# Nightmare-n/GD-MAE

Hardware: AMD Instinct MI355X
Metric: MAE pre-train frames/sec (Waymo-shape, 180k pts, 75% mask) (higher is better)
Workload: dtype bf16

## Files before the change

gd-mae_amd/csrc/decoder_blocks.hip:

```cpp
#include "../../include/gdmae_hip.h"
#include "common.h"
#include "dw_grouped.h"
#include <stdlib.h>

typedef float f32x16 __attribute__((ext_vector_type(16)));
typedef __bf16 bf16x8 __attribute__((ext_vector_type(8)));
typedef short s16x4 __attribute__((ext_vector_type(4)));

namespace {

constexpr int kC = 128;
constexpr int kChunk = 64;
constexpr int kXBytes = kChunk * kC * 2;
constexpr int kMaxTok = 2048;
constexpr int kHP = 6;
constexpr int kQ = 32;

template <int U>
struct Geo {
  static constexpr int TPC = kChunk / (U * U);
  static constexpr int HW = U + 2;
  static constexpr int HS = HW * HW;
  static constexpr int LT = U == 4 ? 36 : 24;
  static constexpr int NP = 2;
// ... 291 lines not shown
  GD_REQUIRE(n < (1ll << 31) && H > 0 && W > 0 && H % u == 0 && W % u == 0, "decoder_block_dw: map size");
  hipStream_t st = (hipStream_t)stream;
  BlockDwArgs A{(const unsigned short*)P, a, b, (const unsigned short*)bg, site, (const unsigned short*)dYc, tile_slot, (float*)workspace,
                n, (int)(n / (u * u)), H, W, (H + 7) / 8, (W + 7) / 8, 0, 0};
  block_dw_pick(n, &A.S, &A.cps);
  GD_REQUIRE(A.S % 8 == 0 && block_dw_fits(u, A.cps), "decoder_block_dw: too many tokens per slice (gdmae_decoder_block_dw_workspace_bytes returns 0)");
  {
    GdTimed timed(GD_T_DEC_CONV_BWD, st, (double)n * (2.0 * kC + 2.0 * kC + 4.0) + 36.0 * A.S * kC * kC, 2.0 * n * 9.0 * kC * kC);
    const int rc = u == 4 ? block_dw_launch<4>(A, st) : block_dw_launch<2>(A, st);
    if (rc) return rc;
  }
  hipLaunchKernelGGL(k_block_dw_reduce, dim3(gd_div_up(9ll * kC * kC, 256)), dim3(256), 0, st, (const float*)workspace, A.S, out, ld_out, m_off);
  GD_LAUNCH_CHECK();
  return 0;
}
```

gd-mae_amd/csrc/plan.hip:

```cpp
#include "../../include/gdmae_hip.h"
#include "common.h"
#include <string.h>

int gd_voxelize_impl(const float* points, long long n_points, int n_cols, const float* lo, const float* vs, const int* grid_xyz,
                     int batch_size, float* points_out, long long* point_coords, long long* inverse, int* inverse32,
                     long long* voxel_coords, int* pillar_cell, int* pillar_pt_off, int* pillar_pts, int* point_rank,
                     int* sample_pillar_off, float* pillar_mean, int* cell2pillar_out, int* counts, void* workspace, size_t workspace_bytes,
                     void* lb_state, float* points_pm, int* row_pillar, hipStream_t st);
size_t gd_voxelize_lb_state_bytes(long long n_points, long long cells);
size_t gd_plan_scan_state_bytes(long long n);
size_t gd_plan_win_state_bytes(long long n);
int gd_plan_visible_tokens(const float* mask, const int* cell2pillar, long long n_cells, int* tok_pillar, int* tok_cell, int* map,
                           int* n_tok, void* lb_state, hipStream_t st);
int gd_plan_downsample(const int* map_in, int B, int Yi, int Xi, int* tok_cell_out, int* map_out, int* n_out, void* lb_state,
                       hipStream_t st);
struct Dims {
  int B, Y, X;
};
struct PlanJob {
  const int* n_tok;
  const int* tok_cell;
  Dims dt, dm;
  const int* map;
  int mode, s;
// ... 74 lines not shown
};

int check(const gdmae_plan_params* p) {
  GD_REQUIRE(p != nullptr, "geometry plan: null parameters");
  GD_REQUIRE(p->n_points >= 0 && p->n_points < (1ll << 31) && p->n_cols >= 4 && p->n_cols <= 65 && p->batch_size >= 1,
             "geometry plan: bad point buffer");
  GD_REQUIRE(p->grid[0] >= 1 && p->grid[1] >= 1 && p->grid[2] == 1, "geometry plan: single-layer pillar grids (spt_backbone_mae.py:94)");
  GD_REQUIRE(p->n_stages >= 1 && p->n_stages <= GDMAE_PLAN_MAX_STAGES, "geometry plan: 1..4 stages");
  for (int i = 0; i < p->n_stages; ++i) {
    GD_REQUIRE(p->stride[i] == 1 || p->stride[i] == 2, "geometry plan: conv_down stride 1 or 2 (k3 s2 p1)");
    GD_REQUIRE(i == 0 || p->stride[i] == 2, "geometry plan: only the first stage may keep the resolution");
    GD_REQUIRE(p->win_x[i] >= 1 && p->win_y[i] >= 1 && p->win_x[i] * p->win_y[i] <= 64, "geometry plan: window must fit one wavefront");
    GD_REQUIRE(p->n_levels[i] >= 1 && p->n_levels[i] <= 3, "geometry plan: 1..3 drop levels");
  }
  GD_REQUIRE(p->n_dec >= 0 && p->n_dec <= 3, "geometry plan: at most 3 decoder source stages");
  for (int g = 0; g < p->n_dec; ++g) GD_REQUIRE(p->dec_sources[g] >= 0 && p->dec_sources[g] < p->n_stages, "geometry plan: decoder source");
  return 0;
}

int layout(const gdmae_plan_params* p, gdmae_plan_buffer* table, int max_entries, Offsets& O, size_t* total, int* n_entries) {
  if (int rc = check(p)) return rc;
  Layout L{table, max_entries, 0, 0, true};
  const int B = p->batch_size, gx = p->grid[0], gy = p->grid[1], F = p->n_cols - 1;
  const long long n0 = p->cap_points > p->n_points ? p->cap_points : p->n_points;
  O.cells = (long long)B * gx * gy;
  GD_REQUIRE(O.cells < (1ll << 31), "geometry plan: B*Y*X must fit int32");
  O.cap_pts = n0 > 0 ? n0 : 1;
  O.m_cap = n0 < O.cells ? n0 : O.cells;
  if (O.m_cap < 1) O.m_cap = 1;
  const long long cap = O.cap_pts;
// ... 71 lines not shown
    if (g.up_s > 1) O.s[i].up_sites = L.add(name("up_sites"), sizeof(int) * g.cap * g.up_s * g.up_s);
    O.s[i].win_ws = L.add(name("win_ws"), gd_plan_windows_ws_bytes(B, g.Y, g.X, p->win_x[i], p->win_y[i]));
    const long long wcap = g.n_win < g.cap ? g.n_win : g.cap;
    for (int sh = 0; sh < 2; ++sh)
      for (int k = 0; k < 7; ++k) {
        snprintf(nm, sizeof(nm), "s%d.w%d.%s", i, sh, kWin[k]);
        O.s[i].w[sh][k] = L.add(nm, sizeof(int) * (k < 5 ? g.cap : wcap));
      }
  }
  O.dec_slot = O.dec_list = O.dec_flag = -1;
  if (O.dec) {
    O.dec_slot = L.add("dec.tile_slot", sizeof(int) * nt);
    O.dec_list = L.add("dec.tile_list", sizeof(int) * nt);
    O.dec_flag = L.add("dec.flag", sizeof(int) * nt);
    for (int g = 0; g < p->n_dec; ++g) {
      const StageGeo& sg = O.geo[p->dec_sources[g]];
      snprintf(nm, sizeof(nm), "dec.nbr%d", g);
      O.dec_nbr[g] = L.add(nm, sizeof(int) * sg.cap * sg.up_s * sg.up_s * 9);
    }
  }
  GD_REQUIRE(L.ok, "geometry plan: buffer table too small");
  if (total) *total = L.off;
  if (n_entries) *n_entries = L.n;
  return 0;
}

}

extern "C" int gdmae_geometry_plan_layout(const gdmae_plan_params* p, gdmae_plan_buffer* table, int max_entries, int* n_entries,
                                          size_t* total_bytes) {
// ... 88 lines not shown
    int rc = gd_plan_jobs(J, cap_max, st);
    if (rc) return rc;
    rc = gd_plan_windows_all(W, ns, st);
    if (rc) return rc;
  }
  if (O.dec) {
    const int* maps[3];
    int ups[3];
    for (int g = 0; g < p->n_dec; ++g) {
      maps[g] = I(O.s[p->dec_sources[g]].map);
      ups[g] = O.geo[p->dec_sources[g]].up_s;
    }
    int rc = gd_decoder_tiles_lb(maps, ups, p->n_dec, B, gy, gx, I(O.dec_slot), I(O.dec_list), n_act, I(O.dec_flag), lb, st);
    if (rc) return rc;
    for (int g = 0; g < p->n_dec; ++g) {
      const int si = p->dec_sources[g];
      const StageGeo& sg = O.geo[si];
      const int* sites = sg.up_s > 1 ? I(O.s[si].up_sites) : I(O.s[si].tok_cell);
      rc = gd_decoder_site_rulebook(sites, n_tok + si, sg.up_s * sg.up_s, sg.cap * sg.up_s * sg.up_s, I(O.dec_slot), gy, gx, I(O.dec_nbr[g]), st);
      if (rc) return rc;
    }
  }
  return 0;
}
```

gd-mae_amd/gdmae_hip/decoder.py:

```python
from __future__ import annotations

import torch
import torch.nn.functional as F

import os

from . import bn as gbn
from . import lib as L
from . import ops, packing
from . import plan as gplan
from . import timing

CONV_BWD = os.environ.get("GDMAE_DEC_BWD", "implicit")
BLOCK_BWD = os.environ.get("GDMAE_DEC_BLOCK", "1")

BN_EPS, BN_MOM = 1e-3, 0.01



def colstats(x2d: torch.Tensor):
    R, C = x2d.shape
    assert x2d.is_contiguous() and x2d.dtype in (torch.float32, torch.bfloat16)
    out = torch.empty(2 * C, dtype=torch.float64, device=x2d.device)
    ws = torch.empty(L.load().gdmae_colstats_workspace_bytes(C), dtype=torch.uint8, device=x2d.device)
    L.call("gdmae_colstats", L.ptr(x2d), R, C, int(x2d.dtype == torch.bfloat16), L.ptr(out), L.ptr(ws), L.stream())
    return out[:C], out[C:]


def _gather_slice(table2d, idx, col0, ncol):
# ... 186 lines not shown
            S = tap_region @ regD
            Wk = conv_w.permute(2, 3, 0, 1).reshape(9, C2, Cin)
            tot = torch.einsum('ko,koi->i', S, Wk.double()).contiguous()
            dWk = (S[:, :, None] * bgz.double()[None, None, :]).float()
            Wd = Wk.to(cdt)
        grads = [None] * 7
        dW_rows = []
        col = 0
        implicit = None
        if (CONV_BWD == "implicit" and tile_slot is not None and y2.dtype == torch.bfloat16 and use_native and C2 == 128
                and all(w == 128 for w in ctx.widths) and len(ctx.geom) > 6 and ctx.geom[6] is not None):
            dt = ctx.geom[6][0]
            packed = packing.decoder_conv_packed(ctx.conv_param, ctx.widths, ctx.direct_w is not None)
            if packed is not None:
                if dt.nbr is None:
                    dt.nbr = gplan.decoder_site_rulebooks(dt, sites, ctx.geom[6][2])
                dYc = torch.empty_like(y2)
                L.call("gdmae_decoder_dy", L.ptr(y2), L.ptr(dt.tile_list), dt.n_act, L.ptr(k01), L.ptr(k01[C2:]), L.ptr(rows),
                       L.ptr(cell2pillar), H, W, C2, L.ptr(dYc), L.stream())
                implicit = (dt, packed, dYc)
        for i, w in enumerate(ctx.widths):
            P = Ps[i]
            n = P.shape[0]
            ab = ab_l[i]
            if implicit is not None:
                dt, packed, dYc = implicit
                nbr = dt.nbr[i]
                assert nbr.shape[0] == n, (nbr.shape, n)
                dX = torch.empty(n, w, dtype=cdt, device=dev)
                L.call("gdmae_spconv", L.ptr(dYc), 0, L.ptr(nbr), packed.data_ptr() + i * 9 * w * C2 * 2, n, C2, w, L.ptr(dX), 8, L.stream())
                bg = bgz[col:col + w]
                u = int(ctx.geom[6][2][i])
                ws_block = 0
                if BLOCK_BWD != "0" and u in (2, 4) and P.dtype == torch.bfloat16 and P.is_contiguous() and sites[i].numel() >= n:
                    ws_block = int(L.load().gdmae_decoder_block_dw_workspace_bytes(n, u))
                if ws_block > 0:
                    ws = torch.empty(ws_block, dtype=torch.uint8, device=dev)
                    L.call("gdmae_decoder_block_dw", L.ptr(P), L.ptr(ab), L.ptr(ab[w:]), L.ptr(bg), L.ptr(sites[i]), n, u, L.ptr(dYc),
                           L.ptr(tile_slot), H, W, L.ptr(dWk), Cin, col, L.ptr(ws), L.stream())
                else:
                    n_pad = int(L.load().gdmae_tap_dw_rows(n, w, C2))
                    Zd = torch.empty(n_pad, w, dtype=cdt, device=dev)
                    L.call("gdmae_rows_affine_relu_sub", L.ptr(P), _bf(P), None, n, w, L.ptr(ab), L.ptr(ab[w:]), L.ptr(bg), L.ptr(Zd),
                           _bf(Zd), w, 0, L.stream())
                    ws = torch.empty(L.load().gdmae_tap_dw_workspace_bytes(n, w, C2), dtype=torch.uint8, device=dev)
                    L.call("gdmae_tap_dw", L.ptr(Zd), n, n_pad, w, L.ptr(dYc), L.ptr(nbr), C2, L.ptr(dWk), Cin, col, L.ptr(ws), L.stream())
            else:
                G = torch.empty(n, 9 * C2, dtype=cdt, device=dev)
                with timing.kernel("k_conv_grad_taps", 2.0 * n * 9 * C2 * G.element_size()):
                    L.call("gdmae_conv3x3_grad_taps", L.ptr(y2), _bf(y2), L.ptr(tile_slot), L.ptr(ybg), L.ptr(k01), L.ptr(k01[C2:]),
# ... 145 lines not shown
        return stage_plan.tok_cell
    pre = getattr(stage_plan, "_up_sites", None)
    if pre is not None and pre[0] == s and stage_plan.Y * s == Y and stage_plan.X * s == X:
        return pre[1]
    return gplan.upsample_cells(stage_plan.tok_cell, stage_plan.Y, stage_plan.X, s).reshape(-1).contiguous()


def sparse_decoder(model_cfg, deblocks, conv_out, hidden, pillar_cell, cell2pillar, B, Y, X, want_dense=False, conv_impl='tiles', pre_conv_hook=None):
    R = B * Y * X
    args, bns = [], []
    cdt = torch.bfloat16 if torch.is_autocast_enabled() else torch.float32
    src_idx = [int(src[-1]) - 1 for src in model_cfg.FEATURES_SOURCE]
    tiles = None
    if cdt == torch.bfloat16 and conv_impl == 'tiles':
        ep = hidden[0]._plan
        dt = gplan.decoder_tiles(ep, src_idx, Y, X)
        tiles = (dt, [hidden[i].stage_plan.map for i in src_idx], [Y // hidden[i].stage_plan.Y for i in src_idx])
    for i, src in enumerate(model_cfg.FEATURES_SOURCE):
        h = hidden[int(src[-1]) - 1]
        sp = h.stage_plan
        deconv, bn = deblocks[i][0], deblocks[i][1]
        s = int(deconv.stride[0])
        assert deconv.kernel_size == (s, s) and sp.Y * s == Y and sp.X * s == X and deconv.bias is None
        P = deconv_rows(h.features, deconv)
        args += [upsampled_sites(sp, s, Y, X), P, bn.weight, bn.bias]
        bns.append(bn)
    conv, bn2 = conv_out[0], conv_out[1]
    outs = DecoderHead.apply((B, Y, X, bns[0].eps, bn2.eps, cdt, tiles, pre_conv_hook), conv.weight, bn2.weight, bn2.bias, pillar_cell,
                             cell2pillar, tuple(bns) + (bn2,), *args)
    out, y2, mean2, var2 = outs[:4]
    dense = None
# ... 22 lines not shown
```

gd-mae_amd/gdmae_hip/lib.py:

```python
from __future__ import annotations

import ctypes as C
import os

import torch

_HERE = os.path.dirname(os.path.abspath(__file__))
LIB_PATH = os.path.abspath(os.path.join(_HERE, "..", "csrc", "libgdmae_hip.so"))
if os.environ.get("GDMAE_LIB"):
    LIB_PATH = os.path.abspath(os.environ["GDMAE_LIB"])


class GdmaeHipError(RuntimeError):
    pass


_P, _I, _L, _F, _D, _Z = C.c_void_p, C.c_int, C.c_longlong, C.c_float, C.c_double, C.c_size_t

SIGNATURES = {
    "gdmae_abi_version": (_I, []),
    "gdmae_target_arch": (C.c_char_p, []),
    "gdmae_last_error": (C.c_char_p, []),
    "gdmae_voxelize_workspace_bytes": (_Z, [_L, _I, _I, _I, _I]),
    "gdmae_voxelize": (_I, [_P, _L, _I, _P, _P, _P, _I, _P, _P, _P, _P, _P, _P, _P, _P, _P, _P, _P, _P, _P, _P, _Z, _P]),
# ... 94 lines not shown
    "gdmae_gemm_tn_splitk": (_I, [_P, _P, _P, _L, _I, _I, _I, _I, _P, _P]),
    "gdmae_conv_block_scratch_bytes": (_Z, [_L, _L, _I, _I, _I]),
    "gdmae_spconv_packed_bytes": (_Z, [_I, _I]),
    "gdmae_spconv_pack_jobs": (_I, [_P, _I, _I, _I, _P, _P]),
    "gdmae_spconv": (_I, [_P, _I, _P, _P, _L, _I, _I, _P, _I, _P]),
    "gdmae_spconv_bias_relu": (_I, [_P, _I, _P, _P, _P, _L, _I, _I, _P, _P]),
    "gdmae_spconv_stat_rows": (_I, [_I, _I, _I]),
    "gdmae_spconv_stats": (_I, [_P, _I, _P, _P, _L, _I, _I, _P, _P, _P]),
    "gdmae_decoder_dy": (_I, [_P, _P, _I, _P, _P, _P, _P, _I, _I, _I, _P, _P]),
    "gdmae_decoder_site_rulebook": (_I, [_P, _P, _I, _L, _P, _I, _I, _P, _P]),
    "gdmae_tap_dw_rows": (_L, [_L, _I, _I]),
    "gdmae_tap_dw_workspace_bytes": (_Z, [_L, _I, _I]),
    "gdmae_tap_dw": (_I, [_P, _L, _L, _I, _P, _P, _I, _P, _I, _I, _P, _P]),
    "gdmae_decoder_block_dw_workspace_bytes": (_Z, [_L, _I]),
    "gdmae_decoder_block_dw": (_I, [_P, _P, _P, _P, _P, _L, _I, _P, _P, _I, _I, _P, _I, _I, _P, _P]),
    "gdmae_conv_block_fwd": (_I, [_P, _P]),
    "gdmae_conv_block_bwd": (_I, [_P, _P]),
    "gdmae_encoder_layer_bytes": (_I, [_L, _I, _I, _I, _I, _P, _P, _P]),
    "gdmae_dw_gemm_workspace_bytes": (_Z, [_L, _I, _I]),
    "gdmae_dw_gemm": (_I, [_P, _P, _L, _I, _I, _P, _P, _P, _P]),
    "gdmae_layer_packed_bytes": (_Z, [_I, _I]),
    "gdmae_layer_pack_jobs": (_I, [_P, _P, _P, _P, _I, _I, _P, _P]),
    "gdmae_layer_pack_job_count": (_I, [_I, _I]),
    "gdmae_tok_gemm_pack": (_I, [_P, _I, _P]),
    "gdmae_tok_gemm": (_I, [_P, _P, _P, _L, _L, _I, _I, _I, _P, _P, _P, _P, _P, _P, _F, _P, _P, _P, _P, _P, _P, _P]),
    "gdmae_tok_gemm_qkv": (_I, [_P, _P, _P, _P, _P, _L, _I, _P, _P, _P]),
    "gdmae_tok_gemm_ffn": (_I, [_P, _P, _P, _P, _P, _L, _L, _I, _P, _P, _P, _P, _F, _P, _P, _P, _P, _P, _P, _P, _P]),
    "gdmae_tok_gemm_ln_bwd_rows": (_I, [_I]),
    "gdmae_tok_gemm_ln_bwd": (_I, [_P, _P, _L, _L, _I, _I, _P, _P, _P, _P, _P, _P, _P, _P, _P, _P]),
    "gdmae_encoder_layer_fwd": (_I, [_P, _P]),
# ... 61 lines not shown
}

class LayerArgs(C.Structure):
    _fields_ = ([("n", _L), ("d", _I), ("ff", _I), ("nhead", _I), ("bf16", _I), ("eps", _F), ("tau_min", _F), ("n_levels", _I),
                 ("n_win", _I * 4), ("max_tokens", _I * 4)]
                + [(k, _P) for k in ("tok_pos", "csr_tok", "win_start", "win_len", "pos_table", "Win", "bin", "Wo", "bo", "W1", "b1",
                                     "W2", "b2", "g1", "be1", "g2", "be2", "tau", "x", "y", "dy", "dx", "dWin", "dbin", "dtau", "dWo",
                                     "dbo", "dW1", "db1", "dW2", "db2", "dg1", "dbe1", "dg2", "dbe2", "saved", "scratch", "packed")]
                + [("x_bf16", _I), ("res_out", _P), ("dres", _P), ("dx_bf16", _P), ("path", _I)])


class PlanParams(C.Structure):
    _fields_ = [("n_points", _L), ("n_cols", _I), ("batch_size", _I), ("lo", _F * 3), ("vs", _F * 3), ("grid", _I * 3), ("n_stages", _I),
                ("stride", _I * 4), ("win_x", _I * 4), ("win_y", _I * 4), ("n_levels", _I * 4), ("drop_lo", (_I * 3) * 4),
                ("drop_hi", (_I * 3) * 4), ("max_tokens", (_I * 3) * 4), ("masked", _I), ("keep_frac", _D), ("n_dec", _I),
                ("dec_sources", _I * 4), ("want_pm", _I), ("cap_points", _L)]


class PlanBuffer(C.Structure):
    _fields_ = [("name", C.c_char * 40), ("offset", _L), ("bytes", _L)]


class ConvBlockArgs(C.Structure):
    _fields_ = ([("n_in", _L), ("n_out", _L), ("cin", _I), ("cout", _I), ("bf16", _I), ("x_f32", _I), ("g_f32", _I),
                 ("eps", _F), ("momentum", _F)]
                + [(k, _P) for k in ("x", "nbr", "nbr_t", "W", "gamma", "beta", "running_mean", "running_var", "num_batches", "cols",
                                     "y", "stats", "ab", "mv", "out", "g", "dx", "dW", "dgamma", "dbeta", "scratch", "packed_fwd", "packed_bwd")]
                + [("out_f32", _I)])


_lib = None
# ... 65 lines not shown
```

gd-mae_amd/gdmae_hip/plan.py:

```python
from __future__ import annotations

from dataclasses import dataclass, field
from typing import List, Optional

import torch

from . import lib as L

I32 = torch.int32


def _empty(n, dtype, dev):
    return torch.empty(int(n), dtype=dtype, device=dev)


@dataclass
class VoxelPlan:
    batch_size: int
    grid: tuple
    lo: tuple
    vs: tuple
    n_cols: int
    N: int
    M: int
# ... 133 lines not shown
    hi = [int(d[k]["drop_range"][1]) for k in keys]
    T = [int(d[k]["max_tokens"]) for k in keys]
    return lo, hi, T


def _decoder_tiles_launch(maps, ups, B, H, W, dev) -> dict:
    nt = B * ((H + 7) // 8) * ((W + 7) // 8)
    r = dict(tile_slot=_empty(nt, I32, dev), tile_list=_empty(nt, I32, dev), n_act=_empty(1, I32, dev), B=B, H=H, W=W)
    ws = _empty(L.load().gdmae_decoder_tiles_workspace_bytes(B, H, W), torch.uint8, dev)
    L.call("gdmae_decoder_tiles", L.host_ptrs(maps), L.host_i32(ups), len(maps), B, H, W, L.ptr(r["tile_slot"]),
           L.ptr(r["tile_list"]), L.ptr(r["n_act"]), L.ptr(ws), L.stream())
    r["_ws"] = ws
    return r


def decoder_tiles(ep: "EncoderPlan", sources, H: int, W: int) -> DecoderTiles:
    sources = tuple(int(v) for v in sources)
    dt = ep.dec_tiles
    if dt is not None and dt.sources == sources and dt.H == H and dt.W == W:
        return dt
    st = [ep.stages[i] for i in sources]
    B = st[0].B
    ups = [H // sp.Y for sp in st]
    assert all(sp.Y * u == H and sp.X * u == W for sp, u in zip(st, ups))
    r = _decoder_tiles_launch([sp.map for sp in st], ups, B, H, W, st[0].map.device)
    n = int(r["n_act"].item())
    ep.dec_tiles = DecoderTiles(sources, B, H, W, n, r["tile_slot"], r["tile_list"][:n], _site_rulebooks(st, ups, r["tile_slot"], H, W))
    return ep.dec_tiles


def decoder_site_rulebooks(dt: "DecoderTiles", sites, ups):
    out = []
    for st, u in zip(sites, ups):
        n_dev = torch.tensor([st.numel() // (u * u)], dtype=I32, device=st.device)
        nbr = _empty(st.numel() * 9, I32, st.device)
        L.call("gdmae_decoder_site_rulebook", L.ptr(st.contiguous()), L.ptr(n_dev), u * u, st.numel(), L.ptr(dt.tile_slot), dt.H, dt.W,
               L.ptr(nbr), L.stream())
        out.append(nbr.view(-1, 9))
    return out


def _site_rulebooks(stages, ups, tile_slot, H, W):
    out = []
    for sp, u in zip(stages, ups):
        sites = sp.tok_cell if u == 1 else (sp._up_sites[1] if getattr(sp, "_up_sites", None) is not None and sp._up_sites[0] == u
                                            else upsample_cells(sp.tok_cell, sp.Y, sp.X, u).reshape(-1).contiguous())
        n_dev = torch.tensor([sp.n_tok], dtype=I32, device=tile_slot.device)
        nbr = _empty(sites.numel() * 9, I32, tile_slot.device)
        L.call("gdmae_decoder_site_rulebook", L.ptr(sites.contiguous()), L.ptr(n_dev), u * u, sites.numel(), L.ptr(tile_slot), H, W, L.ptr(nbr),
               L.stream())
        out.append(nbr.view(-1, 9))
    return out


def _encoder_launch(vox, m_cap: int, strides, window_shapes, drop_infos, keep_frac, noise, dec_sources=None) -> dict:
    if isinstance(vox, dict):
        dev, grid, B = vox["src"].device, vox["grid"], vox["batch_size"]
        sample_off, pillar_cell, vcounts = vox["sample_off"], vox["pillar_cell"], vox["counts"]
    else:
# ... 124 lines not shown
    e = _encoder_launch(vox, vox.M, strides, window_shapes, drop_infos, keep_frac, noise, dec_sources)
    return _encoder_finalize(e, e["counts"].tolist(), vox.M)


import collections
import time as _time

EVENT_WAIT_S = 0.0

_PLAN_SHAPES = collections.OrderedDict()
_PLAN_SHAPES_MAX = 32
_PLAN_GRANULE = 16384
_PINNED = {}


def _plan_shape(n0, ncols, B, pcr, voxel_size, grid_size, strides, window_shapes, drop_infos, keep_frac, dec_sources):
    gx, gy, gz = (int(g) for g in grid_size)
    lo = tuple(float(v) for v in pcr[:3])
    vs = tuple(float(v) for v in voxel_size)
    drops = tuple(tuple(map(tuple, _drop_arrays(d))) for d in drop_infos)
    n_exact = n0
    n0 = max(1, (n0 + _PLAN_GRANULE - 1) // _PLAN_GRANULE) * _PLAN_GRANULE
    key = (n0, ncols, B, lo, vs, (gx, gy, gz), tuple(int(s) for s in strides), tuple(tuple(int(v) for v in w) for w in window_shapes),
           drops, None if keep_frac is None else float(keep_frac), None if dec_sources is None else tuple(int(i) for i in dec_sources))
    hit = _PLAN_SHAPES.get(key)
    if hit is not None:
        _PLAN_SHAPES.move_to_end(key)
        return hit
    del n_exact
    import ctypes as C
    ns = len(strides)
    assert gz == 1, "the SST backbone works on single-layer pillar grids (spt_backbone_mae.py:94)"
    assert 1 <= ns <= 4
    P = L.PlanParams()
    P.n_points, P.cap_points, P.n_cols, P.batch_size = n0, n0, ncols, B
    for i in range(3):
        P.lo[i], P.vs[i] = lo[i], vs[i]
        P.grid[i] = (gx, gy, gz)[i]
    P.n_stages = ns
# ... 10 lines not shown
        for l in range(len(dT)):
            P.drop_lo[i][l], P.drop_hi[i][l], P.max_tokens[i][l] = dlo[l], dhi[l], dT[l]
        cap_in = cap
        if int(strides[i]) > 1:
            assert int(strides[i]) == 2, "only the k3 s2 p1 strided sparse conv of the shipped configs is implemented"
            Y, X = (Y - 1) // 2 + 1, (X - 1) // 2 + 1
            cap = min(4 * cap, B * Y * X)
        us = gy // Y
        up_s = us if (us >= 1 and us * Y == gy and us * X == gx) else 0
        geo.append(dict(Y=Y, X=X, cap=cap, cap_in=cap_in, up_s=up_s, strided=int(strides[i]) > 1, T=list(dT)))
    P.masked = int(keep_frac is not None)
    P.keep_frac = float(keep_frac) if keep_frac is not None else 1.0
    P.n_dec = 0 if dec_sources is None else len(dec_sources)
    for g in range(P.n_dec):
        P.dec_sources[g] = int(dec_sources[g])
    P.want_pm = 1
    table = (L.PlanBuffer * 160)()
    n_ent, total = C.c_int(0), C.c_size_t(0)
    L.call("gdmae_geometry_plan_layout", C.byref(P), table, 160, C.byref(n_ent), C.byref(total))
    names = {table[i].name.decode(): (int(table[i].offset), int(table[i].bytes)) for i in range(n_ent.value)}
    hit = _PLAN_SHAPES[key] = (P, names, int(total.value), geo, m_cap, (lo, vs, (gx, gy, gz)))
    while len(_PLAN_SHAPES) > _PLAN_SHAPES_MAX:
        _PLAN_SHAPES.popitem(last=False)
    return hit


class _Arena:

    def __init__(self, raw, names):
        self.raw, self.names = raw, names
# ... 6 lines not shown
        off, _ = self.names[name]
        es = 8 if dtype == torch.int64 else 4
        strides, acc = [], 1
        for d in reversed(shape):
            strides.append(acc)
            acc *= int(d)
        return self.base[dtype].as_strided(tuple(int(d) for d in shape), tuple(reversed(strides)), off // es)


class PlanPrefetch:

    _side = {}
    _arena_bytes = {}

    def __init__(self, points, point_cloud_range, voxel_size, grid_size, batch_size, strides, window_shapes, drop_infos,
                 keep_frac=None, noise=None, ready=None, dec_sources=None):
        import ctypes as C
        assert points.is_cuda and points.dtype == torch.float32 and points.dim() == 2
        points = points.contiguous()
        dev = points.device
        main = torch.cuda.current_stream(dev)
        side = PlanPrefetch._side.setdefault(dev.index, torch.cuda.Stream(device=dev))
        side.wait_stream(main)
        if ready is not None:
            side.wait_event(ready)
        points.record_stream(side)
        if noise is not None:
            noise.record_stream(side)
        n0, ncols = points.shape
        P, names, total, geo, m_cap, _ = self.shape = _plan_shape(n0, ncols, int(batch_size), point_cloud_range, voxel_size, grid_size,
                                                                    strides, window_shapes, drop_infos, keep_frac, dec_sources)
        self.masked, self.dec_sources, self.batch_size, self.ncols = keep_frac is not None, dec_sources, int(batch_size), ncols
        with torch.cuda.stream(side):
            cap = PlanPrefetch._arena_bytes.get(dev.index, 0)
            if total > cap:
                cap = PlanPrefetch._arena_bytes[dev.index] = -(-total // (64 << 20)) * (64 << 20)
            raw = torch.empty(cap, dtype=torch.uint8, device=dev)
            if self.masked and noise is None:
                noise = torch.rand(m_cap, device=dev, dtype=torch.float32)
            if noise is not None:
                assert noise.dtype == torch.float32 and noise.numel() >= 1
                noise = noise.contiguous()
            Pc = L.PlanParams.from_buffer_copy(P)
            Pc.n_points = n0
            L.call("gdmae_geometry_plan", C.byref(Pc), L.ptr(points), None if noise is None else L.ptr(noise), L.ptr(raw), total, L.stream())
            self.arena = _Arena(raw, names)
# ... 47 lines not shown
                wpre = f"{pre}w{k}."
                wps.append(WindowPlan(V(wpre + "tok_win", i32, n), V(wpre + "tok_level", i32, n), V(wpre + "tok_slot", i32, n),
                                      V(wpre + "tok_pos", i32, n), V(wpre + "csr_tok", i32, n), V(wpre + "win_start", i32, nw),
                                      V(wpre + "win_len", i32, nw), [int(v) for v in wc[0:3]], [int(v) for v in wc[3:6]], list(g["T"])))
            n_prev = (int(c[2 + i - 1]) if i > 0 else n_vis) if g["strided"] else 0
            sp = StagePlan(B, g["Y"], g["X"], n, V(pre + "tok_cell", i32, n), V(pre + "map", i32, B * g["Y"] * g["X"]),
                           V(pre + "nbr_subm", i32, n, 9), V(pre + "nbr_down", i32, n, 9) if g["strided"] else None,
                           V(pre + "nbr_down_t", i32, n_prev, 9) if g["strided"] else None, wps)
            sp._nbr_subm_t = V(pre + "nbr_subm_t", i32, n, 9)
            sp._up_sites = (g["up_s"], V(pre + "up_sites", i32, n * g["up_s"] * g["up_s"])) if g["up_s"] > 1 else None
            stages.append(sp)
        dt = None
        if A.has("dec.tile_slot"):
            n_act = int(c[2 + ns + 16 * ns])
            nt = B * ((gy + 7) // 8) * ((gx + 7) // 8)
            nbrs = [V(f"dec.nbr{g}", i32, stages[int(si)].n_tok * geo[int(si)]["up_s"] ** 2, 9) for g, si in enumerate(self.dec_sources)]
            dt = DecoderTiles(tuple(int(i) for i in self.dec_sources), B, gy, gx, n_act, V("dec.tile_slot", i32, nt), V("dec.tile_list", i32, n_act),
                              nbrs)
        ep = EncoderPlan(V("mask", f32, M) if self.masked else None, V("tok_pillar", i32, stages[0].n_tok if not geo[0]["strided"] else n_vis),
                         stages, dt)
        self.arena = self.points = self.keep = None
        return vox, ep


def _tensors_of(obj):
    out = []
    if isinstance(obj, torch.Tensor):
        if obj.is_cuda:
            out.append(obj)
    elif isinstance(obj, dict):
        for v in obj.values():
# ... 6 lines not shown
```

gd-mae_amd/pcdet/models/backbones_3d/spt_backbone_mae.py:

```python
import torch
import torch.nn as nn

from .spt_backbone import SSTBlockV1, build_decoder, run_decoder, stage_plan_args
from ...utils.spconv_utils import SparseConvTensor
from gdmae_hip import decoder as gdec, ops, plan as gplan


def _only_the_pred_head_sees_the_gradient(pred) -> bool:
    fn = pred.grad_fn
    if fn is None or not type(fn).__name__.startswith('ViewBackward') or pred._backward_hooks or pred.retains_grad:
        return False
    nxt = [f for f, _ in fn.next_functions if f is not None]
    if len(nxt) != 1 or 'PredHeadFn' not in type(nxt[0]).__name__:
        return False
    return not getattr(nxt[0], '_tensor_pre_hooks', None) and not getattr(nxt[0], '_pre_hooks', None) and not getattr(nxt[0], '_retains_grad_hooks', None)


class _DeferredPlan:
    __slots__ = ("_mod", "_args", "_pf")

    def __init__(self, mod, args):
        self._mod, self._args, self._pf = mod, args, None

    def __call__(self):
# ... 77 lines not shown
            sf = run_decoder(self.model_cfg, self.decoder_deblocks, self.decoder_conv_out, hidden)
            assert sf.shape[0] == B and sf.shape[2] == Y and sf.shape[3] == X
            pyramid = ops.GatherUnique.apply(sf.permute(0, 2, 3, 1).reshape(B * Y * X, sf.shape[1]), vox.pillar_cell)
        src0 = self.model_cfg.FEATURES_SOURCE[0]
        batch_dict.update({'encoded_spconv_tensor': hidden[-1], 'encoded_spconv_tensor_stride': Y0 // hidden[-1].spatial_shape[0],
                           'multi_scale_3d_features': feats, 'multi_scale_3d_strides': strides, 'spatial_features': sf,
                           'spatial_features_stride': strides[src0] // self.model_cfg.FUSE_LAYER[src0].UPSAMPLE_STRIDE})
        batch_dict.update({'voxel_features': pyramid, 'voxel_coords': all_coords,
                           'voxel_shuffle_inds': torch.arange(all_coords.shape[0], device=all_coords.device)})
        self.forward_ret_dict = self.target_assigner(batch_dict)
        return batch_dict

    def prefetch_plan(self, points, batch_size, noise=None, ready=None):
        return gplan.PlanPrefetch(points, self.point_cloud_range, self.voxel_size, self.grid_size, int(batch_size),
                                  *stage_plan_args(self.model_cfg.SST_BLOCK_LIST), keep_frac=1 - self.mask_ratio, noise=noise,
                                  ready=ready, dec_sources=self._dec_sources())

    def prefetch_plan_under_decoder(self, points, batch_size, noise=None, ready=None):
        self._pre_conv_hook = d = _DeferredPlan(self, (points, batch_size, noise, ready))
        return d

    def _dec_sources(self):
        if self.decoder_impl != 'sparse' or self.decoder_conv_impl != 'tiles':
            return None
        return [int(src[-1]) - 1 for src in self.model_cfg.FEATURES_SOURCE]

    def target_assigner(self, batch_dict):
        vox = batch_dict['_gdmae_vox']
        gt = ops.group_gt_points(vox, self.mask_cfg.NUM_GT_POINTS)
        flat = gdec.pred_head(batch_dict['voxel_features'], self.decoder_pred)
        return {'pred_points': flat.view(vox.M, -1, 3), 'gt_points': gt, 'mask': batch_dict['voxel_mae_mask'],
                'pred_lazy_scale': bool(getattr(flat, '_gd_pred_head', False))}
```

include/gdmae_hip.h:

```cpp
#ifndef GDMAE_HIP_H
#define GDMAE_HIP_H

#include <stddef.h>
#include <stdint.h>

#ifdef __cplusplus
extern "C" {
#endif

int gdmae_abi_version(void);
const char* gdmae_target_arch(void);
const char* gdmae_last_error(void);

size_t gdmae_voxelize_workspace_bytes(long long n_points, int batch_size, int gx, int gy, int gz);
int gdmae_voxelize(const float* points, long long n_points, int n_cols, const float* lo, const float* vs,
                   const int* grid_xyz, int batch_size, float* points_out, long long* point_coords,
                   long long* inverse, int* inverse32, long long* voxel_coords, int* pillar_cell,
                   int* pillar_pt_off, int* pillar_pts, int* point_rank, int* sample_pillar_off,
                   float* pillar_mean, int* cell2pillar, int* counts, void* workspace, size_t workspace_bytes,
                   void* stream);

int gdmae_decorate_points(const float* points, const long long* point_coords, const int* inverse32,
                          const float* pillar_mean, long long N, int n_cols, const float* lo, const float* vs,
                          float* out, void* stream);
// ... 222 lines not shown
int gdmae_spconv_stat_rows(int cin, int cout, int x_f32);
int gdmae_spconv_stats(const void* X, int x_f32, const int* nbr, const void* packed, long long n, int cin, int cout, void* Y, float* part,
                       void* stream);
int gdmae_decoder_dy(const void* Yc, const int* tile_list, int n_act, const float* k0, const float* k1, const float* rows,
                     const int* cell2pillar, int H, int W, int C, void* dYc, void* stream);
int gdmae_decoder_site_rulebook(const int* site, const int* n_dev, int sites_per_tok, long long cap_sites, const int* tile_slot,
                                int H, int W, int* nbr, void* stream);
long long gdmae_tap_dw_rows(long long n, int M, int N);
size_t gdmae_tap_dw_workspace_bytes(long long n, int M, int N);
int gdmae_tap_dw(const void* G, long long n, long long n_pad, int M, const void* X, const int* nbr, int N, float* out, int ld_out,
                 int m_off, void* workspace, void* stream);
size_t gdmae_decoder_block_dw_workspace_bytes(long long n, int u);
int gdmae_decoder_block_dw(const void* P, const float* a, const float* b, const void* bg, const int* site, long long n, int u,
                           const void* dYc, const int* tile_slot, int H, int W, float* out, int ld_out, int m_off, void* workspace,
                           void* stream);
int gdmae_conv_block_fwd(const gdmae_conv_block_args* args , void* stream);
int gdmae_conv_block_bwd(const gdmae_conv_block_args* args , void* stream);

typedef struct gdmae_layer_args {
  long long n;
  int d, ff, nhead, bf16;
  float eps, tau_min;
  int n_levels;
  int n_win[4], max_tokens[4];
  const int* tok_pos;
  const int* csr_tok;
  const int* win_start;
  const int* win_len;
  const float* pos_table;
  const void *Win, *bin, *Wo, *bo, *W1, *b1, *W2, *b2;
// ... 110 lines not shown
  long long n_points;
  int n_cols, batch_size;
  float lo[3], vs[3];
  int grid[3];
  int n_stages;
  int stride[GDMAE_PLAN_MAX_STAGES];
  int win_x[GDMAE_PLAN_MAX_STAGES], win_y[GDMAE_PLAN_MAX_STAGES];
  int n_levels[GDMAE_PLAN_MAX_STAGES];
  int drop_lo[GDMAE_PLAN_MAX_STAGES][3], drop_hi[GDMAE_PLAN_MAX_STAGES][3], max_tokens[GDMAE_PLAN_MAX_STAGES][3];
  int masked;
  double keep_frac;
  int n_dec;
  int dec_sources[GDMAE_PLAN_MAX_STAGES];
  int want_pm;
  long long cap_points;
} gdmae_plan_params;
typedef struct gdmae_plan_buffer {
  char name[40];
  long long offset, bytes;
} gdmae_plan_buffer;
int gdmae_geometry_plan_layout(const gdmae_plan_params* p, gdmae_plan_buffer* table, int max_entries, int* n_entries,
                               size_t* total_bytes);
int gdmae_geometry_plan(const gdmae_plan_params* p, const float* points, const float* noise, void* arena, size_t arena_bytes,
                        void* stream);

size_t gdmae_center_head_targets_workspace_bytes(int B, int num_max_objs);
int gdmae_center_head_targets(const float* gt_boxes, int B, int n_max, int box_dim, const int* class_map, int n_class_total,
                              int n_cls, const float* pc_range , const float* voxel_size ,
                              float feature_map_stride, int fw, int fh, int num_max_objs, double gaussian_overlap, int min_radius,
                              float* heatmap, float* ret_boxes, long long* inds, long long* mask, void* workspace, void* stream);
// ... 83 lines not shown
```

Baseline: 1057.

## Add halo-tiled block dX kernel for stride-4 decoder conv backward, skip its rulebook

Adds a persistent MFMA kernel that computes the decoder conv input gradient for stride-4 upsampled sources. It stages each token's (u+2)^2 dY halo into LDS and runs all 9 taps from there, with a register ring of weight fragments and pipelined row gathers. This replaces the rulebook-driven gdmae_spconv gather, so the geometry plan no longer builds or allocates the 9-neighbour rulebook for those sources (dec_nbr_skip). Other strides fall back to spconv with a lazily built rulebook. The cost is a more complex kernel with heavy LDS use and new plan/ABI struct fields.

```diff
diff --git a/gd-mae_amd/csrc/decoder_blocks.hip b/gd-mae_amd/csrc/decoder_blocks.hip
--- a/gd-mae_amd/csrc/decoder_blocks.hip
+++ b/gd-mae_amd/csrc/decoder_blocks.hip
@@ -329,3 +329,255 @@
   GD_LAUNCH_CHECK();
   return 0;
 }
+
+namespace {
+
+union SpFragX {
+  uint4 q;
+  bf16x8 v;
+};
+
+template <int U, int ROWS>
+struct GeoX {
+  static constexpr int UU = U * U;
+  static constexpr int TPT = ROWS / UU;
+  static constexpr int HW = U + 2, HS = HW * HW;
+  static constexpr int HR = TPT * HS;
+  static constexpr int NP = HR * 16 / 512;
+  static constexpr int HaloBytes = HR * 256;
+  static constexpr int SP = kC * 2 + 16;
+  static constexpr int Lds = HaloBytes + 2 * HR * 4 + 2 * TPT * 16;
+  static constexpr int NPW = ROWS / 64;
+  static constexpr int BOff = (32 / UU) * HS * 256;
+  static constexpr int Occ = 2 * Lds <= 160 * 1024 ? 2 : 1;
+  static_assert(HR * 16 % 512 == 0 && HR <= 512 && ROWS * SP <= HaloBytes, "tile shape");
+};
+
+struct BlockDxArgs {
+  const unsigned short* dY;
+  const int* site;
+  const int* tile_slot;
+  const uint4* Wp;
+  unsigned short* dZ;
+  long long n;
+  int ntok, ntiles, H, W, TH, TW;
+};
+
+#ifndef GD_DX_RING
+#define GD_DX_RING 4
+#endif
+
+template <int U, int ROWS>
+__global__ __launch_bounds__(512) __attribute__((amdgpu_waves_per_eu(2 * GeoX<U, ROWS>::Occ, 2 * GeoX<U, ROWS>::Occ))) void k_decoder_block_dx(BlockDxArgs A) {
+  using G = GeoX<U, ROWS>;
+  constexpr int KS = kC / 16, MB = kC / 32, RING = GD_DX_RING, NPW = G::NPW;
+  static_assert(KS % RING == 0, "a tap is whole turns of the ring");
+  extern __shared__ __align__(16) unsigned char lds[];
+  int* rowidx = reinterpret_cast<int*>(lds + G::HaloBytes);
+  int4* tokinfo = reinterpret_cast<int4*>(lds + G::HaloBytes + 2 * G::HR * 4);
+  const int tid = threadIdx.x, lane = tid & 63, wv = __builtin_amdgcn_readfirstlane(tid >> 6);
+  const int mb0 = wv >> 1, nb0 = (wv & 1) * NPW;
+  const uint4* __restrict__ wp = A.Wp + (size_t)mb0 * 64;
+  const int grid = (int)gridDim.x;
+  auto tile_of = [&](int j) { return (int)blockIdx.x + j * grid; };
+
+  SpFragX wr[RING];
+#pragma unroll
+  for (int g = 0; g < RING; ++g) wr[g].q = wp[(size_t)g * MB * 64 + lane];
+
+  int tt = tid;
+  auto fresh = [&]() { asm volatile("" : "+v"(tt)); };
+  int tsv = 0;
+  bool tval = false;
+  auto tok_a = [&](int j) {
+    if (tid < G::TPT) {
+      const long long tok = (long long)tile_of(j) * G::TPT + tid;
+      tval = tok < A.ntok;
+      tsv = A.site[(tval ? tok : A.ntok - 1) * G::UU];
+    }
+  };
+  auto tok_b = [&](int j) {
+    if (tid < G::TPT) {
+      const int x0 = tsv % A.W, r = tsv / A.W;
+      tokinfo[(j & 1) * G::TPT + tt] = make_int4(r / A.H, tval ? r % A.H : -(1 << 20), x0, 0);
+    }
+  };
+  int slotv = -1, locv = -1;
+  auto resolve_a = [&](int j) {
+    if (tid < G::HR) {
+      const int tl = tt / G::HS, rem = tt - tl * G::HS;
+      const int hy = rem / G::HW, hx = rem - hy * G::HW;
+      const int4 t = tokinfo[(j & 1) * G::TPT + tl];
+      const int yy = t.y + hy - 1, xx = t.z + hx - 1;
+      const bool in = yy >= 0 && yy < A.H && xx >= 0 && xx < A.W;
+      slotv = A.tile_slot[in ? (t.x * A.TH + (yy >> 3)) * A.TW + (xx >> 3) : 0];
+      locv = in ? (yy & 7) * 8 + (xx & 7) : -1;
+    }
+  };
+  auto resolve_b = [&](int j) {
+    if (tid < G::HR) rowidx[(j & 1) * G::HR + tt] = (locv >= 0 && slotv >= 0) ? slotv * 64 + locv : -1;
+  };
+    uint4 rq[G::NP];
+  unsigned keep = 0u;
+  auto load_rows = [&](int j) {
+    unsigned k = 0u;
+#pragma unroll
+    for (int p = 0; p < G::NP; ++p) {
+      const int rix = rowidx[(j & 1) * G::HR + p * 32 + (tt >> 4)];
+      const bool ok = rix >= 0;
+      const long long row = ok ? rix : 0;
+      k |= ok ? 1u << p : 0u;
+      rq[p] = *reinterpret_cast<const uint4*>(A.dY + row * kC + (tt & 15) * 8);
+    }
+    keep = k;
+  };
+  auto stage = [&]() {
+#pragma unroll
+    for (int p = 0; p < G::NP; ++p) {
+      const int hr = p * 32 + (tt >> 4), ch = tt & 15;
+      const int tl = hr / G::HS, rem = hr - tl * G::HS;
+      const int hy = rem / G::HW, hx = rem - hy * G::HW;
+      const int f = U == 4 ? 4 * hy + hx : 4 * (tl & 3) + 2 * hy + hx;
+      const unsigned m = ((keep >> p) & 1u) ? 0xFFFFFFFFu : 0u;
+      uint4 q = rq[p];
+      q.x &= m; q.y &= m; q.z &= m; q.w &= m;
+      *reinterpret_cast<uint4*>(lds + hr * 256 + (((ch ^ f) & 15) << 4)) = q;
+    }
+  };
+
+  tok_a(0); tok_b(0);
+  tok_a(1); tok_b(1);
+  __syncthreads();
+  resolve_a(0); resolve_b(0);
+  resolve_a(1); resolve_b(1);
+  __syncthreads();
+  tok_a(2); tok_b(2);
+  load_rows(0);
+
+  for (int j = 0; tile_of(j) < A.ntiles; ++j) {
+    fresh();
+    stage();
+    __syncthreads();
+    fresh();
+    load_rows(j + 1);
+    resolve_a(j + 2);
+    tok_a(j + 3);
+    __builtin_amdgcn_sched_barrier(0);
+
+    f32x16 acc[NPW];
+#pragma unroll
+    for (int b = 0; b < NPW; ++b)
+#pragma unroll
+      for (int i = 0; i < 16; ++i) acc[b][i] = 0.f;
+    const uint4* wq = wp;
+    asm volatile("" : "+s"(wq));
+    fresh();
+    const int l5 = tt & 31, h = (tt >> 5) & 1;
+    int hyc, hxc, rowc, fk = 0;
+    if (U == 4) {
+      hyc = ((l5 >> 2) & 3) + 1;
+      hxc = (l5 & 3) + 1;
+      rowc = (nb0 * 2 + (l5 >> 4)) * G::HS + hyc * G::HW + hxc;
+    } else {
+      const int tl = nb0 * 8 + (l5 >> 2);
+      hyc = ((l5 >> 1) & 1) + 1;
+      hxc = (l5 & 1) + 1;
+      rowc = tl * G::HS + hyc * G::HW + hxc;
+      fk = 4 * (tl & 3);
+    }
+
+#pragma unroll 1
+    for (int tap = 0; tap < 9; ++tap) {
+      const int oy = tap / 3 - 1, ox = tap - (oy + 1) * 3 - 1;
+      const int hy = hyc - oy, hx = hxc - ox;
+      const int f = U == 4 ? 4 * hy + hx : fk + 2 * hy + hx;
+      const int pg = (rowc - (oy * G::HW + ox)) * 256 + (((h ^ f) & 15) << 4);
+      const uint4* wt = wq + (size_t)tap * KS * MB * 64;
+      const uint4* wn = tap == 8 ? wq : wt + (size_t)KS * MB * 64;
+      SpFragX sf[2][NPW];
+#pragma unroll
+      for (int b = 0; b < NPW; ++b) sf[0][b].q = *reinterpret_cast<const uint4*>(lds + pg + b * G::BOff);
+#pragma unroll
+      for (int ks = 0; ks < KS; ++ks) {
+        if (ks + 1 < KS) {
+#pragma unroll
+          for (int b = 0; b < NPW; ++b) sf[(ks + 1) & 1][b].q = *reinterpret_cast<const uint4*>(lds + (pg ^ ((ks + 1) * 32)) + b * G::BOff);
+        }
+#pragma unroll
+        for (int b = 0; b < NPW; ++b) acc[b] = __builtin_amdgcn_mfma_f32_32x32x16_bf16(wr[ks % RING].v, sf[ks & 1][b].v, acc[b], 0, 0, 0);
+        wr[ks % RING].q = ks + RING < KS ? wt[(size_t)(ks + RING) * MB * 64 + lane] : wn[(size_t)(ks + RING - KS) * MB * 64 + lane];
+        __builtin_amdgcn_sched_barrier(0);
+      }
+    }
+    __syncthreads();
+
+    fresh();
+    {
+      const int l5 = tt & 31, h = (tt >> 5) & 1;
+      const int cb = mb0 * 32 + 4 * h;
+#pragma unroll
+      for (int b = 0; b < NPW; ++b) {
+        const int row = (nb0 + b) * 32 + l5;
+#pragma unroll
+        for (int q = 0; q < 4; ++q) {
+          uint2 o;
+          o.x = gd_pack_bf16(acc[b][4 * q], acc[b][4 * q + 1]);
+          o.y = gd_pack_bf16(acc[b][4 * q + 2], acc[b][4 * q + 3]);
+          *reinterpret_cast<uint2*>(lds + row * G::SP + (cb + 8 * q) * 2) = o;
+        }
+      }
+    }
+    resolve_b(j + 2);
+    tok_b(j + 3);
+    __syncthreads();
+    fresh();
+    {
+      const int ch = tt & 15;
+      const long long row0 = (long long)tile_of(j) * ROWS;
+#pragma unroll
+      for (int p = 0; p < ROWS / 32; ++p) {
+        const int rl = p * 32 + (tt >> 4);
+        if (row0 + rl < A.n) *reinterpret_cast<uint4*>(A.dZ + (row0 + rl) * kC + ch * 8) = *reinterpret_cast<const uint4*>(lds + rl * G::SP + ch * 16);
+      }
+    }
+    __syncthreads();
+  }
+}
+
+#ifndef GD_DX_ROWS_U2
+#define GD_DX_ROWS_U2 64
+#endif
+
+template <int U, int ROWS>
+int block_dx_launch(BlockDxArgs A, int max_wgs, hipStream_t st) {
+  using G = GeoX<U, ROWS>;
+  static bool once = false;
+  if (!once) {
+    GD_CHECK(hipFuncSetAttribute((const void*)k_decoder_block_dx<U, ROWS>, hipFuncAttributeMaxDynamicSharedMemorySize, G::Lds));
+    once = true;
+  }
+  A.ntiles = (int)gd_div_up(A.n, ROWS);
+  int slots = 256 * G::Occ;
+  if (max_wgs > 0 && max_wgs < slots) slots = max_wgs;
+  const int tpw = (A.ntiles + slots - 1) / slots;
+  const int grid = (A.ntiles + tpw - 1) / tpw;
+  hipLaunchKernelGGL((k_decoder_block_dx<U, ROWS>), dim3((unsigned)grid), dim3(512), G::Lds, st, A);
+  GD_LAUNCH_CHECK();
+  return 0;
+}
+
+}
+
+extern "C" int gdmae_decoder_block_dx(const void* dYc, const int* site, long long n, int u, const int* tile_slot, int H, int W,
+                                      const void* packed, void* dZ, int max_workgroups, void* stream) {
+  GD_REQUIRE(u == 2 || u == 4, "decoder_block_dx: u must be 2 or 4");
+  GD_REQUIRE(n >= 0 && n % (u * u) == 0, "decoder_block_dx: rows must be whole tokens (u * u sites each)");
+  if (n == 0) return 0;
+  GD_REQUIRE(n < (1ll << 31) && H > 0 && W > 0 && H % u == 0 && W % u == 0, "decoder_block_dx: map size");
+  hipStream_t st = (hipStream_t)stream;
+  BlockDxArgs A{(const unsigned short*)dYc, site, tile_slot, (const uint4*)packed, (unsigned short*)dZ, n, (int)(n / (u * u)), 0, H, W,
+                (H + 7) / 8, (W + 7) / 8};
+  GdTimed timed(GD_T_DEC_CONV_BWD, st, (double)n / (u * u) * ((u + 2.0) * (u + 2.0) * 2.0 * kC + 4.0) + 2.0 * n * kC + 18.0 * kC * kC,
+                2.0 * n * 9.0 * kC * kC);
+  return u == 4 ? block_dx_launch<4, 128>(A, max_workgroups, st) : block_dx_launch<2, GD_DX_ROWS_U2>(A, max_workgroups, st);
+}
diff --git a/gd-mae_amd/csrc/plan.hip b/gd-mae_amd/csrc/plan.hip
--- a/gd-mae_amd/csrc/plan.hip
+++ b/gd-mae_amd/csrc/plan.hip
@@ -112,6 +112,7 @@
     GD_REQUIRE(p->n_levels[i] >= 1 && p->n_levels[i] <= 3, "geometry plan: 1..3 drop levels");
   }
   GD_REQUIRE(p->n_dec >= 0 && p->n_dec <= 3, "geometry plan: at most 3 decoder source stages");
+  GD_REQUIRE(p->dec_nbr_skip >= 0 && p->dec_nbr_skip < 8, "geometry plan: dec_nbr_skip is a mask over the decoder sources");
   for (int g = 0; g < p->n_dec; ++g) GD_REQUIRE(p->dec_sources[g] >= 0 && p->dec_sources[g] < p->n_stages, "geometry plan: decoder source");
   return 0;
 }
@@ -213,6 +214,8 @@
     O.dec_list = L.add("dec.tile_list", sizeof(int) * nt);
     O.dec_flag = L.add("dec.flag", sizeof(int) * nt);
     for (int g = 0; g < p->n_dec; ++g) {
+      O.dec_nbr[g] = -1;
+      if ((p->dec_nbr_skip >> g) & 1) continue;
       const StageGeo& sg = O.geo[p->dec_sources[g]];
       snprintf(nm, sizeof(nm), "dec.nbr%d", g);
       O.dec_nbr[g] = L.add(nm, sizeof(int) * sg.cap * sg.up_s * sg.up_s * 9);
@@ -331,6 +334,7 @@
     int rc = gd_decoder_tiles_lb(maps, ups, p->n_dec, B, gy, gx, I(O.dec_slot), I(O.dec_list), n_act, I(O.dec_flag), lb, st);
     if (rc) return rc;
     for (int g = 0; g < p->n_dec; ++g) {
+      if (O.dec_nbr[g] < 0) continue;
       const int si = p->dec_sources[g];
       const StageGeo& sg = O.geo[si];
       const int* sites = sg.up_s > 1 ? I(O.s[si].up_sites) : I(O.s[si].tok_cell);
diff --git a/gd-mae_amd/gdmae_hip/decoder.py b/gd-mae_amd/gdmae_hip/decoder.py
--- a/gd-mae_amd/gdmae_hip/decoder.py
+++ b/gd-mae_amd/gdmae_hip/decoder.py
@@ -13,6 +13,14 @@
 
 CONV_BWD = os.environ.get("GDMAE_DEC_BWD", "implicit")
 BLOCK_BWD = os.environ.get("GDMAE_DEC_BLOCK", "1")
+BLOCK_DX_STRIDES = (4,)
+
+
+def rulebook_sources(sources, ups):
+    if BLOCK_BWD != "1":
+        return [int(s) for s in sources]
+    return [int(s) for s, u in zip(sources, ups) if int(u) not in BLOCK_DX_STRIDES]
+
 
 BN_EPS, BN_MOM = 1e-3, 0.01
 
@@ -229,7 +237,7 @@
             packed = packing.decoder_conv_packed(ctx.conv_param, ctx.widths, ctx.direct_w is not None)
             if packed is not None:
                 if dt.nbr is None:
-                    dt.nbr = gplan.decoder_site_rulebooks(dt, sites, ctx.geom[6][2])
+                    dt.nbr = [None] * k
                 dYc = torch.empty_like(y2)
                 L.call("gdmae_decoder_dy", L.ptr(y2), L.ptr(dt.tile_list), dt.n_act, L.ptr(k01), L.ptr(k01[C2:]), L.ptr(rows),
                        L.ptr(cell2pillar), H, W, C2, L.ptr(dYc), L.stream())
@@ -240,15 +248,21 @@
             ab = ab_l[i]
             if implicit is not None:
                 dt, packed, dYc = implicit
-                nbr = dt.nbr[i]
-                assert nbr.shape[0] == n, (nbr.shape, n)
-                dX = torch.empty(n, w, dtype=cdt, device=dev)
-                L.call("gdmae_spconv", L.ptr(dYc), 0, L.ptr(nbr), packed.data_ptr() + i * 9 * w * C2 * 2, n, C2, w, L.ptr(dX), 8, L.stream())
                 bg = bgz[col:col + w]
                 u = int(ctx.geom[6][2][i])
                 ws_block = 0
                 if BLOCK_BWD != "0" and u in (2, 4) and P.dtype == torch.bfloat16 and P.is_contiguous() and sites[i].numel() >= n:
                     ws_block = int(L.load().gdmae_decoder_block_dw_workspace_bytes(n, u))
+                dX = torch.empty(n, w, dtype=cdt, device=dev)
+                if ws_block > 0 and BLOCK_BWD != "dw" and u in BLOCK_DX_STRIDES:
+                    L.call("gdmae_decoder_block_dx", L.ptr(dYc), L.ptr(sites[i]), n, u, L.ptr(tile_slot), H, W,
+                           packed.data_ptr() + i * 9 * w * C2 * 2, L.ptr(dX), 0, L.stream())
+                else:
+                    if dt.nbr[i] is None:
+                        dt.nbr[i] = gplan.decoder_site_rulebooks(dt, [sites[i]], [u])[0]
+                    nbr = dt.nbr[i]
+                    assert nbr.shape[0] == n, (nbr.shape, n)
+                    L.call("gdmae_spconv", L.ptr(dYc), 0, L.ptr(nbr), packed.data_ptr() + i * 9 * w * C2 * 2, n, C2, w, L.ptr(dX), 8, L.stream())
                 if ws_block > 0:
                     ws = torch.empty(ws_block, dtype=torch.uint8, device=dev)
                     L.call("gdmae_decoder_block_dw", L.ptr(P), L.ptr(ab), L.ptr(ab[w:]), L.ptr(bg), L.ptr(sites[i]), n, u, L.ptr(dYc),
@@ -424,7 +438,8 @@
     tiles = None
     if cdt == torch.bfloat16 and conv_impl == 'tiles':
         ep = hidden[0]._plan
-        dt = gplan.decoder_tiles(ep, src_idx, Y, X)
+        ups = [Y // hidden[i].stage_plan.Y for i in src_idx]
+        dt = gplan.decoder_tiles(ep, src_idx, Y, X, nbr_sources=rulebook_sources(src_idx, ups))
         tiles = (dt, [hidden[i].stage_plan.map for i in src_idx], [Y // hidden[i].stage_plan.Y for i in src_idx])
     for i, src in enumerate(model_cfg.FEATURES_SOURCE):
         h = hidden[int(src[-1]) - 1]
diff --git a/gd-mae_amd/gdmae_hip/lib.py b/gd-mae_amd/gdmae_hip/lib.py
--- a/gd-mae_amd/gdmae_hip/lib.py
+++ b/gd-mae_amd/gdmae_hip/lib.py
@@ -132,6 +132,7 @@
     "gdmae_tap_dw": (_I, [_P, _L, _L, _I, _P, _P, _I, _P, _I, _I, _P, _P]),
     "gdmae_decoder_block_dw_workspace_bytes": (_Z, [_L, _I]),
     "gdmae_decoder_block_dw": (_I, [_P, _P, _P, _P, _P, _L, _I, _P, _P, _I, _I, _P, _I, _I, _P, _P]),
+    "gdmae_decoder_block_dx": (_I, [_P, _P, _L, _I, _P, _I, _I, _P, _P, _I, _P]),
     "gdmae_conv_block_fwd": (_I, [_P, _P]),
     "gdmae_conv_block_bwd": (_I, [_P, _P]),
     "gdmae_encoder_layer_bytes": (_I, [_L, _I, _I, _I, _I, _P, _P, _P]),
@@ -223,7 +224,7 @@
     _fields_ = [("n_points", _L), ("n_cols", _I), ("batch_size", _I), ("lo", _F * 3), ("vs", _F * 3), ("grid", _I * 3), ("n_stages", _I),
                 ("stride", _I * 4), ("win_x", _I * 4), ("win_y", _I * 4), ("n_levels", _I * 4), ("drop_lo", (_I * 3) * 4),
                 ("drop_hi", (_I * 3) * 4), ("max_tokens", (_I * 3) * 4), ("masked", _I), ("keep_frac", _D), ("n_dec", _I),
-                ("dec_sources", _I * 4), ("want_pm", _I), ("cap_points", _L)]
+                ("dec_sources", _I * 4), ("want_pm", _I), ("cap_points", _L), ("dec_nbr_skip", _I)]
 
 
 class PlanBuffer(C.Structure):
diff --git a/gd-mae_amd/gdmae_hip/plan.py b/gd-mae_amd/gdmae_hip/plan.py
--- a/gd-mae_amd/gdmae_hip/plan.py
+++ b/gd-mae_amd/gdmae_hip/plan.py
@@ -171,7 +171,7 @@
     return r
 
 
-def decoder_tiles(ep: "EncoderPlan", sources, H: int, W: int) -> DecoderTiles:
+def decoder_tiles(ep: "EncoderPlan", sources, H: int, W: int, nbr_sources=None) -> DecoderTiles:
     sources = tuple(int(v) for v in sources)
     dt = ep.dec_tiles
     if dt is not None and dt.sources == sources and dt.H == H and dt.W == W:
@@ -182,7 +182,7 @@
     assert all(sp.Y * u == H and sp.X * u == W for sp, u in zip(st, ups))
     r = _decoder_tiles_launch([sp.map for sp in st], ups, B, H, W, st[0].map.device)
     n = int(r["n_act"].item())
-    ep.dec_tiles = DecoderTiles(sources, B, H, W, n, r["tile_slot"], r["tile_list"][:n], _site_rulebooks(st, ups, r["tile_slot"], H, W))
+    ep.dec_tiles = DecoderTiles(sources, B, H, W, n, r["tile_slot"], r["tile_list"][:n], _site_rulebooks(st, ups, r["tile_slot"], H, W, _nbr_wanted(sources, nbr_sources)))
     return ep.dec_tiles
 
 
@@ -197,9 +197,20 @@
     return out
 
 
-def _site_rulebooks(stages, ups, tile_slot, H, W):
+def _nbr_wanted(sources, nbr_sources):
+    if nbr_sources is None:
+        return [True] * len(sources)
+    want = set(int(i) for i in nbr_sources)
+    assert want <= set(int(i) for i in sources), (nbr_sources, sources)
+    return [int(i) in want for i in sources]
+
+
+def _site_rulebooks(stages, ups, tile_slot, H, W, wanted=None):
     out = []
-    for sp, u in zip(stages, ups):
+    for g, (sp, u) in enumerate(zip(stages, ups)):
+        if wanted is not None and not wanted[g]:
+            out.append(None)
+            continue
         sites = sp.tok_cell if u == 1 else (sp._up_sites[1] if getattr(sp, "_up_sites", None) is not None and sp._up_sites[0] == u
                                             else upsample_cells(sp.tok_cell, sp.Y, sp.X, u).reshape(-1).contiguous())
         n_dev = torch.tensor([sp.n_tok], dtype=I32, device=tile_slot.device)
@@ -354,7 +365,7 @@
 _PINNED = {}
 
 
-def _plan_shape(n0, ncols, B, pcr, voxel_size, grid_size, strides, window_shapes, drop_infos, keep_frac, dec_sources):
+def _plan_shape(n0, ncols, B, pcr, voxel_size, grid_size, strides, window_shapes, drop_infos, keep_frac, dec_sources, nbr_sources=None):
     gx, gy, gz = (int(g) for g in grid_size)
     lo = tuple(float(v) for v in pcr[:3])
     vs = tuple(float(v) for v in voxel_size)
@@ -362,7 +373,8 @@
     n_exact = n0
     n0 = max(1, (n0 + _PLAN_GRANULE - 1) // _PLAN_GRANULE) * _PLAN_GRANULE
     key = (n0, ncols, B, lo, vs, (gx, gy, gz), tuple(int(s) for s in strides), tuple(tuple(int(v) for v in w) for w in window_shapes),
-           drops, None if keep_frac is None else float(keep_frac), None if dec_sources is None else tuple(int(i) for i in dec_sources))
+           drops, None if keep_frac is None else float(keep_frac), None if dec_sources is None else tuple(int(i) for i in dec_sources),
+           None if (dec_sources is None or nbr_sources is None) else tuple(_nbr_wanted(dec_sources, nbr_sources)))
     hit = _PLAN_SHAPES.get(key)
     if hit is not None:
         _PLAN_SHAPES.move_to_end(key)
@@ -403,6 +415,8 @@
     P.n_dec = 0 if dec_sources is None else len(dec_sources)
     for g in range(P.n_dec):
         P.dec_sources[g] = int(dec_sources[g])
+    if dec_sources is not None and nbr_sources is not None:
+        P.dec_nbr_skip = sum(1 << g for g, w in enumerate(_nbr_wanted(dec_sources, nbr_sources)) if not w)
     P.want_pm = 1
     table = (L.PlanBuffer * 160)()
     n_ent, total = C.c_int(0), C.c_size_t(0)
@@ -439,7 +453,7 @@
     _arena_bytes = {}
 
     def __init__(self, points, point_cloud_range, voxel_size, grid_size, batch_size, strides, window_shapes, drop_infos,
-                 keep_frac=None, noise=None, ready=None, dec_sources=None):
+                 keep_frac=None, noise=None, ready=None, dec_sources=None, nbr_sources=None):
         import ctypes as C
         assert points.is_cuda and points.dtype == torch.float32 and points.dim() == 2
         points = points.contiguous()
@@ -454,7 +468,7 @@
             noise.record_stream(side)
         n0, ncols = points.shape
         P, names, total, geo, m_cap, _ = self.shape = _plan_shape(n0, ncols, int(batch_size), point_cloud_range, voxel_size, grid_size,
-                                                                    strides, window_shapes, drop_infos, keep_frac, dec_sources)
+                                                                    strides, window_shapes, drop_infos, keep_frac, dec_sources, nbr_sources)
         self.masked, self.dec_sources, self.batch_size, self.ncols = keep_frac is not None, dec_sources, int(batch_size), ncols
         with torch.cuda.stream(side):
             cap = PlanPrefetch._arena_bytes.get(dev.index, 0)
@@ -532,7 +546,8 @@
         if A.has("dec.tile_slot"):
             n_act = int(c[2 + ns + 16 * ns])
             nt = B * ((gy + 7) // 8) * ((gx + 7) // 8)
-            nbrs = [V(f"dec.nbr{g}", i32, stages[int(si)].n_tok * geo[int(si)]["up_s"] ** 2, 9) for g, si in enumerate(self.dec_sources)]
+            nbrs = [V(f"dec.nbr{g}", i32, stages[int(si)].n_tok * geo[int(si)]["up_s"] ** 2, 9) if A.has(f"dec.nbr{g}") else None
+                    for g, si in enumerate(self.dec_sources)]
             dt = DecoderTiles(tuple(int(i) for i in self.dec_sources), B, gy, gx, n_act, V("dec.tile_slot", i32, nt), V("dec.tile_list", i32, n_act),
                               nbrs)
         ep = EncoderPlan(V("mask", f32, M) if self.masked else None, V("tok_pillar", i32, stages[0].n_tok if not geo[0]["strided"] else n_vis),
diff --git a/gd-mae_amd/pcdet/models/backbones_3d/spt_backbone_mae.py b/gd-mae_amd/pcdet/models/backbones_3d/spt_backbone_mae.py
--- a/gd-mae_amd/pcdet/models/backbones_3d/spt_backbone_mae.py
+++ b/gd-mae_amd/pcdet/models/backbones_3d/spt_backbone_mae.py
@@ -115,7 +115,7 @@
     def prefetch_plan(self, points, batch_size, noise=None, ready=None):
         return gplan.PlanPrefetch(points, self.point_cloud_range, self.voxel_size, self.grid_size, int(batch_size),
                                   *stage_plan_args(self.model_cfg.SST_BLOCK_LIST), keep_frac=1 - self.mask_ratio, noise=noise,
-                                  ready=ready, dec_sources=self._dec_sources())
+                                  ready=ready, dec_sources=self._dec_sources(), nbr_sources=self._dec_nbr_sources())
 
     def prefetch_plan_under_decoder(self, points, batch_size, noise=None, ready=None):
         self._pre_conv_hook = d = _DeferredPlan(self, (points, batch_size, noise, ready))
@@ -126,6 +126,12 @@
             return None
         return [int(src[-1]) - 1 for src in self.model_cfg.FEATURES_SOURCE]
 
+    def _dec_nbr_sources(self):
+        srcs = self._dec_sources()
+        if srcs is None:
+            return None
+        return gdec.rulebook_sources(srcs, [int(self.decoder_deblocks[i][0].stride[0]) for i in range(len(srcs))])
+
     def target_assigner(self, batch_dict):
         vox = batch_dict['_gdmae_vox']
         gt = ops.group_gt_points(vox, self.mask_cfg.NUM_GT_POINTS)
diff --git a/include/gdmae_hip.h b/include/gdmae_hip.h
--- a/include/gdmae_hip.h
+++ b/include/gdmae_hip.h
@@ -260,6 +260,8 @@
 int gdmae_decoder_block_dw(const void* P, const float* a, const float* b, const void* bg, const int* site, long long n, int u,
                            const void* dYc, const int* tile_slot, int H, int W, float* out, int ld_out, int m_off, void* workspace,
                            void* stream);
+int gdmae_decoder_block_dx(const void* dYc, const int* site, long long n, int u, const int* tile_slot, int H, int W, const void* packed,
+                           void* dZ, int max_workgroups, void* stream);
 int gdmae_conv_block_fwd(const gdmae_conv_block_args* args , void* stream);
 int gdmae_conv_block_bwd(const gdmae_conv_block_args* args , void* stream);
 
@@ -400,6 +402,7 @@
   int dec_sources[GDMAE_PLAN_MAX_STAGES];
   int want_pm;
   long long cap_points;
+  int dec_nbr_skip;
 } gdmae_plan_params;
 typedef struct gdmae_plan_buffer {
   char name[40];
```

Result: no change. 1059, median of 6 (+0.2%).
